# cnosdb/cnosdb

Measured on NVIDIA H100. Metric: decoded+aggregated points/s, higher is better.
Workload: dtype i64/f64

## Files before the change

cnosdb_b200/csrc/scan_kernels.cuh:

```cuda
#pragma once
#include <type_traits>

#include "cursors.cuh"

namespace tskv {

constexpr uint32_t FULL = 0xffffffffu;
constexpr int MAX_RANGES = 8;
constexpr int N_TK = 3;
constexpr int N_VK = 3;
constexpr int N_SERIAL_BINS = N_TK * N_VK;
enum { BIN_COOP_RLE_S8B = N_SERIAL_BINS, BIN_COOP_S8B_S8B = N_SERIAL_BINS + 1, BIN_COOP_RLE_GOR = N_SERIAL_BINS + 2,
       BIN_COOP_S8B_GOR = N_SERIAL_BINS + 3 };
constexpr int N_BINS = N_SERIAL_BINS + 4;

enum { TK_RLE = 0, TK_S8B = 1, TK_GEN = 2 };
enum { VK_S8B = 0, VK_GOR = 1, VK_GEN = 2 };

__host__ __device__ inline int time_class(uint8_t dk) {
  return dk == DK_RLE_SC ? TK_RLE : dk == DK_S8B_SC ? TK_S8B : TK_GEN;
}
__host__ __device__ inline int value_class(uint8_t dk) {
  return dk == DK_S8B_ZZ ? VK_S8B : dk == DK_GORILLA ? VK_GOR : VK_GEN;
}
// ... 1123 lines not shown

template <int VK>
__device__ __forceinline__ void flush_runs(const ScanParams &P, uint64_t *stab, uint64_t *stage, uint32_t &seq, bool active,
                                           uint32_t qcol, uint64_t cell, uint8_t pt, uint8_t mask, const ValueAcc<VK> &va) {
  const uint32_t m = __ballot_sync(FULL, active);
  if (m == 0) return;
  const uint32_t lane = threadIdx.x & 31;
  const uint64_t gcell = ((uint64_t)qcol << 32) | (uint32_t)cell;
  const int leader = __ffs(m) - 1;
  const uint64_t lcell = shfl_u64(gcell, leader);
  const bool same = !P.group_by_series && __all_sync(FULL, !active || gcell == lcell);
  if (same) {
    stage_partial<VK>(P, stab, stage, seq, active && va.count, va, (int)lane == leader, lcell);
  } else if (active && va.count) {
    table_update(P, stab, P.cols[qcol], cell, mask, VK == VK_GOR || (VK == VK_GEN && pt == TSKV_PT_F64), va.count, va.sum,
                 va.sum_hi, va.kmin, va.kmax);
  }
}

template <int K, typename S>
__device__ __forceinline__ bool cursor_exhausted(const DeltaCursor<K, S> &c) { return c.exhausted; }
template <bool ZZ>
__device__ __forceinline__ bool cursor_exhausted(const S8bCursor<ZZ> &c) { return c.exhausted(); }
template <int K, typename S>
__device__ __forceinline__ void cursor_reset(DeltaCursor<K, S> &c, uint32_t lane_ring) { c.bs.reset(lane_ring); }
template <bool ZZ>
__device__ __forceinline__ void cursor_reset(S8bCursor<ZZ> &c, uint32_t lane_ring) { c.reset(lane_ring); }

__device__ __forceinline__ uint32_t rle_rows_within(uint64_t d, uint64_t delta, double inv, uint32_t left) {
  const double e = (double)d * inv;
  if (e >= (double)left) return left;
  uint64_t q = (uint64_t)e;
  if (__umul64hi(q, delta) != 0 || q * delta > d) q--;
  else if (d - q * delta >= delta) q++;
  return (uint32_t)min((uint64_t)left, q + 1);
}

template <int TK, int VK, bool SEL>
__device__ __forceinline__ void scan_chunk_seg(const ScanParams &P, uint32_t item_begin, uint32_t item_end,
                                               uint32_t ring_base, uint64_t *stab, uint64_t *stage,
                                               uint32_t part, uint32_t n_parts, uint32_t part_rows) {
  const uint32_t lane = threadIdx.x & 31;
  const uint32_t item = item_begin + lane;
  const bool have_item = item < item_end;
  const uint32_t tslot = ring_base + lane * RING_LANE_STRIDE;
  const uint32_t vslot = ring_base + (TK == TK_S8B ? RING_BYTES_PER_WARP : 0) + lane * RING_LANE_STRIDE;

  uint32_t page = 0, slot = 0, qcol = 0, n_rows = 0;
  uint8_t pt = VK == VK_GOR ? TSKV_PT_F64 : TSKV_PT_I64, mask = 0;
  PageView tpv, vpv;
  S8bCursor<false> tcur;
  uint64_t rle_t0 = 0, rle_delta = 0;
  double rle_inv = 0.0;
  typename std::conditional<VK == VK_S8B, S8bCursor<true>, DeltaCursor<-1, SeqStream>>::type vcur_d;
  GorillaRing vcur_g;
  const uint32_t *vbm = nullptr;
  const uint32_t *keepw = nullptr;
  bool allnull = false;
  int64_t pend_t = 0;
  __shared__ uint4 s_tomb[SCAN_THREADS];

  if (TK == TK_S8B) tcur.reset(tslot);
  if (VK == VK_GOR) vcur_g.reset(vslot);
  else cursor_reset(vcur_d, vslot);
  uint32_t r0 = 0, page_rows = 0;
  if (have_item) {
    page = P.work_page[item];
    slot = P.work_slot[item];
    qcol = P.work_qcol[item] & 0x7f;
    const tskv_page_desc vd = P.descs[page];
    if (P.has_tomb) s_tomb[threadIdx.x] = tomb_lookup(P, vd.series_id, vd.column_id);
    const uint32_t tpage = P.time_page_of[page];
    const tskv_page_desc td = P.descs[tpage];
    if (VK != VK_GOR) pt = P.cols[qcol].phys_type;
    mask = P.cols[qcol].agg_mask;
    page_rows = vd.num_values;
    uint32_t sk_v = SKIP_NONE, sk_t = SKIP_NONE;
    bool split = false;
    if (n_parts > 1 && page_rows > part_rows) {
      sk_v = __ldg(P.skip_off + page);
      sk_t = TK == TK_S8B ? __ldg(P.skip_off + tpage) : 0u;
      split = sk_v != SKIP_NONE && sk_t != SKIP_NONE;
    }
    r0 = part * part_rows;
    tskv_status st = kind_status(vd.reserved);
    if (part != 0 && (!split || r0 >= page_rows)) {
    } else if (st != TSKV_OK) {
      report_error(P, st, page);
    } else {
      tpv.open(P.arena, td);
      vpv.open(P.arena, vd);
      n_rows = split ? min(page_rows, r0 + part_rows) : page_rows;
      vbm = reinterpret_cast<const uint32_t *>(vpv.bitset);
      if (P.row_keep) keepw = P.row_keep + P.keep_off[tpage];
      const uint32_t ent = r0 / SKIP_ROWS - 1;
      if (TK == TK_RLE) {
        DeltaCursor<DK_RLE_SC, BeStream> rc;
        st = rc.open(tpv, td.reserved);
        rle_delta = rc.delta;
        rle_t0 = rc.v + rc.delta;
        if ((int64_t)rle_delta > 0) rle_inv = 1.0 / (double)rle_delta;
      } else if (part == 0) {
        st = tcur.open(tpv, td.reserved, tslot);
      } else {
        tcur.restore(tpv, tslot, load_skip(P.skip + sk_t + ent));
      }
      if (st == TSKV_OK) {
        if (part == 0) {
          if (VK == VK_GOR) vcur_g.open(vpv, vslot);
          else { st = vcur_d.open(vpv, vd.reserved, vslot); allnull = vd.reserved == DK_ALLNULL; }
        } else {
          const SkipEntry e = load_skip(P.skip + sk_v + ent);
          if constexpr (VK == VK_GOR) vcur_g.restore(vpv, vslot, e);
          else if constexpr (VK == VK_S8B) vcur_d.restore(vpv, vslot, e);
        }
      }
      if (st == TSKV_OK && n_rows) {
        if (TK == TK_RLE) pend_t = (int64_t)(rle_t0 + (uint64_t)r0 * rle_delta);
        else if (part == 0) pend_t = (int64_t)tcur.next();
        else pend_t = (int64_t)tcur.v;
      }
      if (st != TSKV_OK) { report_error(P, st, st == TSKV_ERR_BITSET_MISMATCH ? tpage : page); n_rows = 0; }
    }
  }
  const bool to_page_end = n_rows == page_rows;
  ring_drain();

  ValueAcc<VK> va;
  va.reset();
  RunAcc acc;
  acc.first_ts = acc.last_ts = 0; acc.first_val = acc.last_val = 0; acc.first_ok = acc.last_ok = false;
  BucketState bk; bk.valid = false; bk.floor_regime = false; bk.lo = 0; bk.hi = 0; bk.idx = 0;
  bool have_run = false;
  uint32_t run_idx = 0;
  uint32_t row = r0;
  if (n_rows == 0) row = 0;
  uint32_t n_points = 0, n_inrange = 0;
  uint32_t vword = 0, vahead = vbm ? __ldg(vbm + (row >> 5)) : 0;
  uint32_t kword = 0xffffffffu;
  bool first_pending = false;
  const uint64_t flip = pt == TSKV_PT_U64 ? 0x8000000000000000ull : 0ull;
  const uint64_t group_base = P.group_by_series ? (uint64_t)slot * P.n_buckets : 0;
  uint32_t staged = 0;

  auto flush_now = [&](bool flush) {
    if (flush) va.fold(pt);
    if (SEL) {
      if (__any_sync(FULL, flush)) {
        acc.count = va.count; acc.sum = va.sum; acc.sum_hi = va.sum_hi; acc.kmin = va.kmin; acc.kmax = va.kmax;
        warp_flush<SEL>(P, stab, flush, qcol, group_base + run_idx, (int64_t)run_idx, pt, mask, acc, slot);
      }
    } else {
      flush_runs<VK>(P, stab, stage, staged, flush, qcol, group_base + run_idx, pt, mask, va);
    }
  };
  auto row_value = [&](bool accumulate, bool &vv, bool &kept) -> uint64_t {
    if ((row & 31) == 0) {
      vword = vahead;
      vahead = __ldg(vbm + (row >> 5) + 1);
      if (keepw) kword = __ldg(keepw + (row >> 5));
    }
    vv = ((vword >> (row & 31)) & 1) && !allnull;
    kept = (kword >> (row & 31)) & 1;
    uint64_t v = 0;
    if (vv) {
      v = VK == VK_GOR ? vcur_g.next() : vcur_d.next();
      n_points++;
      if (accumulate && kept) { va.count++; va.add(v, pt, flip); }
    }
    return v;
  };
  auto check_values = [&]() {
    const bool bad = VK == VK_GOR ? vcur_g.failed() : cursor_exhausted(vcur_d);
    if (bad) {
      report_error(P, (VK == VK_GOR && vcur_g.overran()) ? TSKV_ERR_SHORT_BLOCK : TSKV_ERR_BITSET_MISMATCH, page);
      n_rows = 0;
      have_run = false;
    }
  };

  uint32_t ra = 0, rb1 = 0, nb = 0xffffffffu, q32 = 0, bidx = 0;
  uint64_t e_off = 0, w_rem = 0;
  bool fast = false;
  if (TK == TK_RLE) {
    bool elig = P.n_ranges <= 1 && !P.has_tomb;
    if (elig && n_rows) {
      const uint64_t span_t = (uint64_t)(page_rows - 1) * rle_delta;
      elig = (int64_t)rle_delta > 0 && __umul64hi((uint64_t)(page_rows - 1), rle_delta) == 0 && span_t < (1ull << 62) &&
             rle_t0 + (1ull << 62) < (1ull << 63) && P.width < ((int64_t)1 << 61);
      if (elig) {
        const int64_t t0 = (int64_t)rle_t0;
        ra = 0;
        rb1 = page_rows;
        if (P.n_ranges == 1) {
          const int64_t a = P.ranges[0].min_ts, b = P.ranges[0].max_ts;
          ra = a <= t0 ? 0u : rle_rows_within((uint64_t)(a - 1) - rle_t0, rle_delta, rle_inv, page_rows);
          rb1 = b < t0 ? 0u : rle_rows_within((uint64_t)b - rle_t0, rle_delta, rle_inv, page_rows);
        }
        ra = min(max(ra, row), n_rows);
        rb1 = min(max(rb1, row), n_rows);
        if (P.width > 0 && ra < rb1) {
          const int64_t tr = (int64_t)(rle_t0 + (uint64_t)ra * rle_delta);
          if ((int64_t)((uint64_t)tr - (uint64_t)P.origin_mod + (uint64_t)P.width) < 0) {
            elig = false;
          } else if (!locate_bucket(P, tr, bk)) {
            report_error(P, TSKV_ERR_BUCKET_RANGE, page);
            n_rows = 0;
          } else {
            bidx = bk.idx;
            nb = rle_rows_within((uint64_t)bk.hi - (uint64_t)tr, rle_delta, rle_inv, 0xffffffffu);
            e_off = (uint64_t)tr + (uint64_t)nb * rle_delta - ((uint64_t)bk.hi + 1);
            q32 = rle_rows_within((uint64_t)P.width, rle_delta, rle_inv, 0xffffffffu) - 1;
            w_rem = (uint64_t)P.width - (uint64_t)q32 * rle_delta;
          }
        }
      }
    }
    fast = __all_sync(FULL, elig);
  }

  if (TK == TK_RLE && VK != VK_GEN && !SEL && fast && P.width > 0 && !P.group_by_series) {
    const bool mine = row < n_rows;
    const uint32_t with_rows = __ballot_sync(FULL, mine);
    const int src = with_rows ? __ffs(with_rows) - 1 : 0;
    const uint64_t t_first = rle_t0 + (uint64_t)row * rle_delta;
    const bool agree = (shfl_u64(rle_delta, src) == rle_delta) & (shfl_u64(t_first, src) == t_first) &
                       (shfl_u64(e_off, src) == e_off) & (__shfl_sync(FULL, row, src) == row) &
                       (__shfl_sync(FULL, n_rows, src) == n_rows) & (__shfl_sync(FULL, ra, src) == ra) &
                       (__shfl_sync(FULL, rb1, src) == rb1) & (__shfl_sync(FULL, bidx, src) == bidx) &
                       (__shfl_sync(FULL, nb, src) == nb) & (__shfl_sync(FULL, qcol, src) == qcol);
    if (with_rows && __all_sync(FULL, !mine || agree)) {
      rle_delta = shfl_u64(rle_delta, src);
      e_off = shfl_u64(e_off, src);
      w_rem = shfl_u64(w_rem, src);
      q32 = __shfl_sync(FULL, q32, src);
      row = __shfl_sync(FULL, row, src);
      ra = __shfl_sync(FULL, ra, src);
      rb1 = __shfl_sync(FULL, rb1, src);
      bidx = __shfl_sync(FULL, bidx, src);
      nb = __shfl_sync(FULL, nb, src);
      const uint64_t col = (uint64_t)__shfl_sync(FULL, qcol, src) << 32;
      uint32_t end = __shfl_sync(FULL, n_rows, src);
      while (row < end) {
        if (n_rows) {
          vword = vahead;
          vahead = __ldg(vbm + (row >> 5) + 1);
          if (keepw) kword = __ldg(keepw + (row >> 5));
        }
        const uint32_t wend = min(row + 32, end);
        const uint32_t m = (n_rows && !allnull) ? vword & (0xffffffffu >> (32 - (wend - row))) : 0u;
        const uint32_t lo = min(max(ra, row), wend) - row, hi = max(min(max(rb1, row), wend) - row, lo);
        const uint32_t take = m & kword & (uint32_t)((1ull << hi) - (1ull << lo));
        const bool dense = __all_sync(FULL, take == m);
        uint32_t r = row;
        while (r < wend) {
          const bool in = r >= ra && r < rb1;
          uint32_t pend = r < ra ? min(ra, wend) : wend;
          if (in) {
            if (nb == 0) {
              do {
                bidx++;
                nb = q32 + (e_off < w_rem ? 1u : 0u);
                e_off = e_off + (uint64_t)nb * rle_delta - (uint64_t)P.width;
              } while (nb == 0);
              if (bidx >= P.n_buckets) {
                if (n_rows) { report_error(P, TSKV_ERR_BUCKET_RANGE, page); n_rows = r; }
                end = r;
                break;
              }
            }
            const uint32_t lim = min(rb1, wend);
            pend = nb < lim - r ? r + nb : lim;
            nb -= pend - r;
          }
          const uint32_t pmask = (uint32_t)((1ull << (pend - row)) - (1ull << (r - row)));
          const uint32_t mp = n_rows ? m & pmask : 0u, tp = take & mp;
          n_points += __popc(mp);
          if (in && n_rows) n_inrange += __popc(kword & pmask);
          va.count += __popc(tp);
          if (dense) {
#pragma unroll 1
            for (uint32_t n = __popc(mp); n; n--) {
              const uint64_t v = VK == VK_GOR ? vcur_g.next() : vcur_d.next();
              va.add(v, pt, flip);
            }
          } else {
#pragma unroll 1
            for (uint32_t b = mp; b; b &= b - 1) {
              const uint64_t v = VK == VK_GOR ? vcur_g.next() : vcur_d.next();
              if (tp & b & (0u - b)) va.add(v, pt, flip);
            }
          }
          r = pend;
          if (n_rows) check_values();
          if (in && (nb == 0 || r == rb1)) {
            va.fold(pt);
            stage_partial<VK>(P, stab, stage, staged, n_rows && va.count, va, lane == 0, col | bidx);
            va.reset();
          }
        }
        row = r;
      }
      row = n_rows;
    }
  }

  const bool align = P.width > 0 && !P.group_by_series;
  bool pending = false;
  uint32_t seg_n = 0, seg_b = 0;
  bool seg_in = false, seg_masked = false;
  int64_t lim_lo = 0, lim_hi = 0;
  for (;;) {
    const bool has = row < n_rows;
    if (!__any_sync(FULL, has || have_run)) break;
    if (has && !pending) {
      pending = true;
      seg_in = false;
      seg_masked = false;
      seg_n = 0;
      if (TK == TK_RLE && fast) {
        if (row < ra) seg_n = ra - row;
        else if (row >= rb1) seg_n = n_rows - row;
        else {
          seg_in = true;
          while (nb == 0) {
            bidx++;
            nb = q32 + (e_off < w_rem ? 1u : 0u);
            e_off = e_off + (uint64_t)nb * rle_delta - (uint64_t)P.width;
          }
          if (bidx >= P.n_buckets) {
            report_error(P, TSKV_ERR_BUCKET_RANGE, page);
            seg_in = false;
            n_rows = row;
            pending = false;
          } else {
            seg_n = min(nb, rb1 - row);
            seg_b = bidx;
            if (P.width > 0) nb -= seg_n;
          }
        }
      } else {
        lim_lo = lim_hi = pend_t;
        seg_in = range_span(P, pend_t, lim_lo, lim_hi);
        if (P.has_tomb) {
          const uint4 tl = s_tomb[threadIdx.x];
          const bool dropped = tomb_span(P.tomb_ranges, P.n_tomb_global, pend_t, lim_lo, lim_hi) |
                               tomb_span(P.tomb_ranges + tl.x, tl.y, pend_t, lim_lo, lim_hi);
          seg_masked = tomb_span(P.tomb_ranges + tl.z, tl.w, pend_t, lim_lo, lim_hi);
          if (dropped) seg_in = false;
        }
        if (seg_in) {
          if (!(bk.valid && pend_t >= bk.lo && pend_t <= bk.hi) && !locate_bucket(P, pend_t, bk)) {
            report_error(P, TSKV_ERR_BUCKET_RANGE, page);
            seg_in = false;
            bk.valid = false;
            lim_lo = lim_hi = pend_t;
          } else {
            lim_lo = lim_lo > bk.lo ? lim_lo : bk.lo;
            lim_hi = lim_hi < bk.hi ? lim_hi : bk.hi;
            seg_b = bk.idx;
          }
        }
        if (TK == TK_RLE) {
          const uint32_t left = n_rows - row;
          if ((int64_t)rle_delta > 0) {
            seg_n = rle_rows_within((uint64_t)lim_hi - (uint64_t)pend_t, rle_delta, rle_inv, left);
          } else {
            int64_t t = pend_t;
            do {
              seg_n++;
              t = (int64_t)((uint64_t)t + rle_delta);
            } while (seg_n < left && t >= lim_lo && t <= lim_hi);
          }
        }
      }
    }
    bool go = pending;
    if (align) {
      const uint32_t bmin = __reduce_min_sync(FULL, (pending && seg_in) ? seg_b : 0xffffffffu);
      go = pending && (!seg_in || seg_b == bmin);
    }
    const bool newrun = go && seg_in && (!have_run || seg_b != run_idx);
    const bool flush = have_run && (newrun || !has);
    flush_now(flush);
    if (flush) have_run = false;
    if (newrun) {
      have_run = true;
      run_idx = seg_b;
      va.reset();
      if (SEL) { acc.first_ok = acc.last_ok = false; first_pending = true; }
    }
    if (go) {
      pending = false;
      const bool accumulate = seg_in && !seg_masked;
      if (TK == TK_RLE) {
        const uint32_t rend = row + seg_n;
        uint32_t r = row;
        while (r < rend) {
          if ((r & 31) == 0) {
            vword = vahead;
            vahead = __ldg(vbm + (r >> 5) + 1);
            if (keepw) kword = __ldg(keepw + (r >> 5));
          }
          const uint32_t off = r & 31;
          const uint32_t span = min(32u - off, rend - r);
          const uint32_t smask = 0xffffffffu >> (32 - span);
          const uint32_t m = allnull ? 0u : ((vword >> off) & smask);
          const uint32_t kb = (kword >> off) & smask;
          n_points += __popc(m);
          if (seg_in) n_inrange += __popc(kb);
          if (!SEL) {
            const uint32_t take = accumulate ? (m & kb) : 0u;
            va.count += __popc(take);
            if (__all_sync(__activemask(), take == m)) {
#pragma unroll 1
              for (uint32_t n = __popc(m); n; n--) {
                const uint64_t v = VK == VK_GOR ? vcur_g.next() : vcur_d.next();
                va.add(v, pt, flip);
              }
            } else {
#pragma unroll 1
              for (uint32_t b = m; b; b &= b - 1) {
                const uint64_t v = VK == VK_GOR ? vcur_g.next() : vcur_d.next();
                if (take & b & (0u - b)) va.add(v, pt, flip);
              }
            }
          } else {
            for (uint32_t j = 0; j < span; j++) {
              bool vv = (m >> j) & 1;
              uint64_t v = 0;
              if (vv) v = VK == VK_GOR ? vcur_g.next() : vcur_d.next();
              vv = vv && !seg_masked;
              if (seg_in && ((kb >> j) & 1)) {
                const int64_t t = (int64_t)(rle_t0 + (uint64_t)(r + j) * rle_delta);
                if (first_pending) { acc.first_ts = t; acc.first_val = vv ? v : 0; acc.first_ok = vv; first_pending = false; }
                acc.last_ts = t;
                acc.last_val = vv ? v : 0;
                acc.last_ok = vv;
                if (vv) { va.count++; va.add(v, pt, flip); }
              }
            }
          }
          r += span;
        }
        row = rend;
        if (!(TK == TK_RLE && fast)) pend_t = (int64_t)(rle_t0 + (uint64_t)rend * rle_delta);
      } else {
        int64_t t = pend_t;
        const uint64_t span = (uint64_t)lim_hi - (uint64_t)lim_lo;
        bool more;
#pragma unroll 1
        do {
          bool vv, kept;
          const uint64_t v = row_value(accumulate, vv, kept);
          if (SEL && seg_in && kept) {
            const bool ok = vv && !seg_masked;
            if (first_pending) { acc.first_ts = t; acc.first_val = ok ? v : 0; acc.first_ok = ok; first_pending = false; }
            acc.last_ts = t;
            acc.last_val = ok ? v : 0;
            acc.last_ok = ok;
          }
          if (seg_in && kept) n_inrange++;
          row++;
          t = (int64_t)tcur.next();
          more = row < n_rows && (uint64_t)t - (uint64_t)lim_lo <= span;
        } while (more);
        pend_t = t;
        if (tcur.exhausted() && row < n_rows) { report_error(P, TSKV_ERR_BITSET_MISMATCH, P.time_page_of[page]); n_rows = row; }
      }
      check_values();
    }
  }
  if (!SEL && staged) {
    reduce_staged<VK>(P, stab, stage, staged);
    staged = 0;
  }
  if (VK == VK_GOR && have_item && n_rows != 0 && to_page_end && vcur_g.consumed_any() && !vcur_g.drain())
    report_error(P, TSKV_ERR_SHORT_BLOCK, page);
  ring_drain();
  n_points = __reduce_add_sync(FULL, n_points);
  n_inrange = __reduce_add_sync(FULL, n_inrange);
  if (lane == 0) {
    if (n_points) atomicAdd(&P.stats[0], (unsigned long long)n_points);
    if (n_inrange) atomicAdd(&P.stats[1], (unsigned long long)n_inrange);
  }
}

#ifndef SCAN_MIN_BLOCKS
#define SCAN_MIN_BLOCKS 4
#endif
__host__ __device__ constexpr int scan_min_blocks(int , bool ) { return SCAN_MIN_BLOCKS; }
__host__ __device__ constexpr uint32_t scan_ring_bytes_per_warp(int tk) {
  return tk == TK_RLE ? RING_BYTES_PER_WARP : tk == TK_S8B ? 2 * RING_BYTES_PER_WARP : 0;
}
__host__ __device__ constexpr uint32_t scan_warp_bytes(int tk) {
  return tk == TK_GEN ? 0 : scan_ring_bytes_per_warp(tk) + FLUSH_STAGE_BYTES;
}
template <int TK, int VK, bool SEL>
__global__ void __launch_bounds__(SCAN_THREADS, scan_min_blocks(TK, SEL)) k_scan_aggregate(const __grid_constant__ ScanParams P, int bin) {
  extern __shared__ __align__(16) uint64_t s_tab[];
  if (P.use_smem) {
    for (uint32_t i = threadIdx.x; i < P.smem_words; i += SCAN_THREADS) s_tab[i] = 0;
    __syncthreads();
    for (uint32_t c = 0; c < P.n_cols; c++) {
      const ColState cs = P.cols[c];
      for (uint32_t i = threadIdx.x; i < (uint32_t)P.n_cells; i += SCAN_THREADS) {
        if (cs.agg_mask & TSKV_AGG_MIN) s_tab[cs.s_min + i] = 0x7fffffffffffffffull;
        if (cs.agg_mask & TSKV_AGG_MAX) s_tab[cs.s_max + i] = 0x8000000000000000ull;
      }
    }
    __syncthreads();
  }
  const uint32_t lane = threadIdx.x & 31;
  uint64_t *warp_area = s_tab + ((P.smem_words + 1) & ~1u) + (size_t)(threadIdx.x >> 5) * (scan_warp_bytes(TK) / 8);
  const uint32_t ring_base = (uint32_t)__cvta_generic_to_shared(warp_area);
  uint64_t *stage = warp_area + scan_ring_bytes_per_warp(TK) / 8;
  const uint32_t begin0 = __ldg(P.bin_cstart + bin), end0 = __ldg(P.bin_cstart + bin + 1);
  const uint32_t n_parts = (TK == TK_GEN || VK == VK_GEN || SEL) ? 1u : P.bin_parts[bin];
  const uint32_t part_rows = P.bin_part_rows[bin];
  const uint32_t n_chunks = ((end0 - begin0 + 31) >> 5) * n_parts;
  for (;;) {
    uint32_t c = 0;
    if (lane == 0) c = atomicAdd(P.task_counter + bin, 1u);
    c = __shfl_sync(FULL, c, 0);
    if (c >= n_chunks) break;
    const uint32_t group = n_parts > 1 ? c / n_parts : c;
    const uint32_t part = c - group * n_parts;
    const uint32_t begin = begin0 + (group << 5);
    const uint32_t end = min(begin + 32, end0);
    if constexpr (TK == TK_GEN) scan_chunk_rows<TK, VK, SEL>(P, begin, end, ring_base, s_tab);
    else scan_chunk_seg<TK, VK, SEL>(P, begin, end, ring_base, s_tab, stage, part, n_parts, part_rows);
  }
  if (P.use_smem) {
    __syncthreads();
    for (uint32_t c = 0; c < P.n_cols; c++) {
      const ColState cs = P.cols[c];
      const bool f64 = cs.phys_type == TSKV_PT_F64;
      for (uint32_t i = threadIdx.x; i < (uint32_t)P.n_cells; i += SCAN_THREADS) {
        const uint64_t cnt = s_tab[cs.s_count + i];
        if (!cnt) continue;
        atomicAdd(reinterpret_cast<unsigned long long *>(P.state + cs.count_off + i), (unsigned long long)cnt);
        if (cs.agg_mask & (TSKV_AGG_SUM | TSKV_AGG_MEAN)) {
          const uint64_t sv = s_tab[cs.s_sum + i];
          if (f64) atomicAdd(reinterpret_cast<double *>(P.state + cs.sum_off + i), __longlong_as_double((long long)sv));
          else add_int_sum(P.state + cs.sum_off + i, P.state + cs.sumhi_off + i, cs.agg_mask, sv,
                           (cs.agg_mask & TSKV_AGG_MEAN) ? (int64_t)s_tab[cs.s_hi + i] : 0);
        }
        if (cs.agg_mask & TSKV_AGG_MIN) atomicMin(reinterpret_cast<long long *>(P.state + cs.min_off + i), (long long)s_tab[cs.s_min + i]);
        if (cs.agg_mask & TSKV_AGG_MAX) atomicMax(reinterpret_cast<long long *>(P.state + cs.max_off + i), (long long)s_tab[cs.s_max + i]);
      }
    }
  }
}

struct StateLayout {
  uint64_t sum_i64_off, sum_i64_len;
  uint64_t sum_f64_off, sum_f64_len;
  uint64_t min_off, min_len;
  uint64_t max_off, max_len;
  uint64_t selval_off, selval_len;
  uint64_t first_pairs_off, first_cells;
  uint64_t last_pairs_off, last_cells;
  uint64_t first_keys_off, last_keys_off;
  uint64_t snap_off;
  uint64_t total;
};

__global__ void k_init_state(uint64_t *state, StateLayout L, unsigned long long *aux, uint32_t aux_words, uint32_t *zero32,
                             uint32_t n_zero32, uint32_t *zero32b, uint32_t n_zero32b) {
  uint64_t i = (uint64_t)blockIdx.x * blockDim.x + threadIdx.x;
  uint64_t stride = (uint64_t)gridDim.x * blockDim.x;
  for (uint64_t k = i; k < aux_words; k += stride) aux[k] = 0;
  for (uint64_t k = i; k < n_zero32; k += stride) zero32[k] = 0;
  for (uint64_t k = i; k < n_zero32b; k += stride) zero32b[k] = 0;
  for (uint64_t k = i; k < L.total; k += stride) {
    uint64_t v = 0;
    if (k >= L.min_off && k < L.min_off + L.min_len) v = 0x7fffffffffffffffull;
    else if (k >= L.max_off && k < L.max_off + L.max_len) v = 0x8000000000000000ull;
    else if (k >= L.first_pairs_off && k < L.first_pairs_off + 2 * L.first_cells) v = ((k - L.first_pairs_off) & 1) ? 0 : 0x7fffffffffffffffull;
    else if (k >= L.last_pairs_off && k < L.last_pairs_off + 2 * L.last_cells) v = ((k - L.last_pairs_off) & 1) ? 0 : 0x8000000000000000ull;
    state[k] = v;
  }
}

struct MeanExport {
  uint64_t lo_off, hi_off, dst_off;
  uint32_t is_signed, pad;
};

__global__ void k_export_pairs(uint64_t *state, StateLayout L, const MeanExport *means, uint32_t n_means,
                               uint64_t n_cells) {
  uint64_t i = (uint64_t)blockIdx.x * blockDim.x + threadIdx.x;
  uint64_t stride = (uint64_t)gridDim.x * blockDim.x;
  for (uint32_t m = 0; m < n_means; m++) {
    const MeanExport me = means[m];
    for (uint64_t k = i; k < n_cells; k += stride) {
      uint64_t lo = state[me.lo_off + k];
      int64_t hi = (int64_t)state[me.hi_off + k];
      double d;
      if (me.is_signed) d = (double)(((__int128)hi << 64) + (__int128)(unsigned __int128)lo);
      else d = (double)(((unsigned __int128)(uint64_t)hi << 64) | (unsigned __int128)lo);
      state[me.dst_off + k] = (uint64_t)__double_as_longlong(d);
    }
  }
  for (uint64_t k = i; k < L.first_cells; k += stride) {
    state[L.first_keys_off + k] = state[L.first_pairs_off + 2 * k];
// ... 151 lines not shown
```

cnosdb_b200/csrc/tskv_gpu.cu:

```cuda
#include <algorithm>
#include <cmath>
#include <atomic>
#include <cstdio>
#include <cstdlib>
#include <cstring>
#include <mutex>
#include <string>
#include <thread>
#include <vector>

#include <cuda_runtime.h>
#include <dlfcn.h>
#include <nccl.h>

#include "host_util.h"
#include "decode_kernels.cuh"
#include "skip_kernels.cuh"
#include "merge_kernels.cuh"

using namespace tskv;

#define CU_TRY(ctx, expr)                                                              \
  do {                                                                                 \
    cudaError_t e__ = (expr);                                                          \
// ... 1152 lines not shown
      }
      if (q->n_time_ranges > 0) {
        int64_t qlo = q->time_ranges[0].min_ts, qhi = q->time_ranges[0].max_ts;
        for (uint32_t k = 1; k < q->n_time_ranges; k++) {
          qlo = std::min(qlo, q->time_ranges[k].min_ts);
          qhi = std::max(qhi, q->time_ranges[k].max_ts);
        }
        lo = std::max(lo, qlo);
        hi = std::min(hi, qhi);
      }
      if (hi < lo) {
        rel_bits = 0;
      } else {
        uint64_t span = (uint64_t)hi - (uint64_t)lo;
        rel_bits = bits_for(span);
        rel_base = lo;
      }
    }
    if (rel_bits + slot_bits > 62) {
      ctx->set_error("first/last across series: (bucket width or time span) x series count does not fit the 62-bit tie-break key");
      delete s;
      return TSKV_ERR_UNSUPPORTED;
    }
  }

  std::vector<ColState> cols(q->n_columns);
  StateLayout &sl = s->sl;
  uint64_t off = 0;
  sl.sum_i64_off = off;
  for (uint32_t c = 0; c < q->n_columns; c++) {
    const tskv_agg_column &qc = q->columns[c];
    cols[c] = ColState{};
    cols[c].column_id = qc.column_id;
    cols[c].phys_type = qc.phys_type;
    cols[c].agg_mask = qc.agg_mask;
    cols[c].count_off = off;
    off += n_cells;
    if ((qc.agg_mask & (TSKV_AGG_SUM | TSKV_AGG_MEAN)) && qc.phys_type != TSKV_PT_F64) {
      cols[c].sum_off = off;
      off += n_cells;
    }
  }
  sl.sum_i64_len = off - sl.sum_i64_off;
  sl.sum_f64_off = off;
  for (uint32_t c = 0; c < q->n_columns; c++)
    if ((q->columns[c].agg_mask & (TSKV_AGG_SUM | TSKV_AGG_MEAN)) && q->columns[c].phys_type == TSKV_PT_F64) {
      cols[c].sum_off = off;
      off += n_cells;
    }
  std::vector<MeanExport> means;
  std::vector<uint64_t> msum_off(q->n_columns, 0);
  for (uint32_t c = 0; c < q->n_columns; c++)
    if ((q->columns[c].agg_mask & TSKV_AGG_MEAN) && q->columns[c].phys_type != TSKV_PT_F64) {
      msum_off[c] = off;
      off += n_cells;
    }
  sl.sum_f64_len = off - sl.sum_f64_off;
  uint64_t n_first = 0, n_last = 0;
  for (uint32_t c = 0; c < q->n_columns; c++) {
    if (q->columns[c].agg_mask & TSKV_AGG_FIRST) n_first += n_cells;
    if (q->columns[c].agg_mask & TSKV_AGG_LAST) n_last += n_cells;
  }
  sl.first_cells = n_first;
  sl.last_cells = n_last;
  sl.min_off = off;
  for (uint32_t c = 0; c < q->n_columns; c++)
    if (q->columns[c].agg_mask & TSKV_AGG_MIN) {
      cols[c].min_off = off;
      off += n_cells;
    }
  sl.first_keys_off = off;
  off += n_first;
  sl.min_len = off - sl.min_off;
  sl.max_off = off;
  for (uint32_t c = 0; c < q->n_columns; c++)
    if (q->columns[c].agg_mask & TSKV_AGG_MAX) {
      cols[c].max_off = off;
      off += n_cells;
    }
  sl.last_keys_off = off;
  off += n_last;
  sl.max_len = off - sl.max_off;
  sl.selval_off = off;
  off += n_first + n_last;
  sl.selval_len = n_first + n_last;
  off = (off + 1) & ~1ull;
  sl.first_pairs_off = off;
  {
    uint64_t o = off;
    for (uint32_t c = 0; c < q->n_columns; c++)
      if (q->columns[c].agg_mask & TSKV_AGG_FIRST) {
        cols[c].first_off = o;
        o += 2 * n_cells;
      }
    off = o;
  }
  sl.last_pairs_off = off;
  {
    uint64_t o = off;
    for (uint32_t c = 0; c < q->n_columns; c++)
      if (q->columns[c].agg_mask & TSKV_AGG_LAST) {
        cols[c].last_off = o;
        o += 2 * n_cells;
      }
    off = o;
  }
  sl.snap_off = off;
  off += n_first + n_last;
  for (uint32_t c = 0; c < q->n_columns; c++)
    if (msum_off[c]) {
      cols[c].sumhi_off = off;
      means.push_back(MeanExport{cols[c].sum_off, off, msum_off[c], q->columns[c].phys_type == TSKV_PT_I64 ? 1u : 0u, 0});
      off += n_cells;
    }
  sl.total = off;

  std::vector<OutCol> outs;
  {
    uint64_t fk = sl.first_keys_off, lk = sl.last_keys_off, fv = sl.selval_off, lv = sl.selval_off + n_first;
    for (uint32_t c = 0; c < q->n_columns; c++) {
      const tskv_agg_column &qc = q->columns[c];
      for (unsigned bit = 0; bit < 7; bit++) {
        unsigned agg = 1u << bit;
        if (!(qc.agg_mask & agg)) continue;
        OutCol oc{};
        oc.count_off = cols[c].count_off;
        oc.agg = (uint8_t)agg;
        oc.phys_type = qc.phys_type;
        switch (agg) {
          case TSKV_AGG_SUM: oc.src_off = cols[c].sum_off; break;
          case TSKV_AGG_MEAN: oc.src_off = msum_off[c] ? msum_off[c] : cols[c].sum_off; break;
          case TSKV_AGG_MIN: oc.src_off = cols[c].min_off; break;
          case TSKV_AGG_MAX: oc.src_off = cols[c].max_off; break;
          case TSKV_AGG_FIRST: oc.src_off = fk; oc.val_off = fv; break;
          case TSKV_AGG_LAST: oc.src_off = lk; oc.val_off = lv; break;
          default: break;
        }
        outs.push_back(oc);
      }
      if (qc.agg_mask & TSKV_AGG_FIRST) { fk += n_cells; fv += n_cells; }
      if (qc.agg_mask & TSKV_AGG_LAST) { lk += n_cells; lv += n_cells; }
    }
  }

  const uint32_t n_items = pages->n_items;
  s->ctx = ctx;
  cudaEventCreate(&s->ev0);
  cudaEventCreate(&s->ev1);
  for (int b = 0; b <= N_BINS; b++) cudaEventCreate(&s->ev_bin[b]);
  for (int b = 0; b < N_BINS; b++) {
    cudaEventCreate(&s->ev_bin_start[b]);
    cudaEventCreate(&s->ev_bin_done[b]);
    cudaEventCreateWithFlags(&s->ev_gather[b], cudaEventDisableTiming);
  }
  s->n_series_sel = q->series_ids ? q->n_series : 0;
  s->n_blocks = (n_items + 1023) / 1024;
  cudaError_t e = cudaSuccess;
  uint64_t h2d = 0;
  if (q->series_ids) {
    e = stream_alloc(ctx, &s->d_series, q->n_series);
    if (e == cudaSuccess && q->n_series)
      e = cudaMemcpyAsync(s->d_series, q->series_ids, (size_t)q->n_series * 4, cudaMemcpyHostToDevice, ctx->stream);
    h2d += (uint64_t)q->n_series * 4;
  }
  if (e == cudaSuccess && q->series_ids) e = stream_alloc(ctx, &s->d_rank_slot, pages->series.size());
  if (e == cudaSuccess) e = stream_alloc(ctx, &s->d_bucket, (size_t)2 * N_BINS * q->n_columns + 1);
  {
    const char *wl = getenv("TSKV_WORKLIST");
    s->worklist_by_items = wl ? wl[0] == 'i' : (uint64_t)pages->n_cg > 32ull * std::max<uint64_t>(1, pages->series.size());
  }
  if (e == cudaSuccess) e = stream_alloc(ctx, &s->d_cg_slot, pages->n_cg);
  if (e == cudaSuccess) e = stream_alloc(ctx, &s->d_item_flag, n_items);
  if (e == cudaSuccess) e = stream_alloc(ctx, &s->d_block_count, s->n_blocks);
  if (e == cudaSuccess) e = stream_alloc(ctx, &s->d_work_page, n_items);
  if (e == cudaSuccess) e = stream_alloc(ctx, &s->d_work_slot, n_items);
  if (e == cudaSuccess) e = stream_alloc(ctx, &s->d_work_qcol, n_items);
  if (e == cudaSuccess) e = stream_alloc(ctx, &s->d_bin_cstart, N_BINS + 2);
  if (e == cudaSuccess) e = stream_alloc(ctx, &s->d_cols, cols.size());
  if (e == cudaSuccess) e = stream_alloc(ctx, &s->d_outs, outs.size());
  s->n_means = (uint32_t)means.size();
  if (e == cudaSuccess) e = stream_alloc(ctx, &s->d_means, means.size());
  if (e == cudaSuccess && !means.empty())
    e = cudaMemcpyAsync(s->d_means, means.data(), means.size() * sizeof(MeanExport), cudaMemcpyHostToDevice, ctx->stream);
  if (e == cudaSuccess) e = stream_alloc(ctx, &s->d_state, sl.total);
  s->preds.n = q->n_predicates;
  for (uint32_t k = 0; k < q->n_predicates; k++) s->preds.p[k] = q->predicates[k];
  if (q->n_predicates) ensure_page_stats(ctx, pages);
  if (e == cudaSuccess && q->n_predicates) e = stream_alloc(ctx, &s->d_row_keep, (size_t)pages->keep_words);
  if (e == cudaSuccess) e = stream_alloc(ctx, reinterpret_cast<unsigned long long **>(&s->d_task_counter), 32);
  if (e == cudaSuccess) e = stream_alloc(ctx, &s->d_values, L.n_out * L.n_cells);
  if (e == cudaSuccess) e = stream_alloc(ctx, &s->d_validity, L.validity_bytes + 8);
  if (e == cudaSuccess) e = cudaMemcpyAsync(s->d_outs, outs.data(), outs.size() * sizeof(OutCol), cudaMemcpyHostToDevice, ctx->stream);
  h2d += cols.size() * sizeof(ColState) + outs.size() * sizeof(OutCol) + means.size() * sizeof(MeanExport) + sizeof(ScanParams);
  if (e != cudaSuccess) {
    ctx->set_error(std::string("scan_prepare: ") + cudaGetErrorString(e));
    free_scan(s);
    return e == cudaErrorMemoryAllocation ? TSKV_ERR_OOM : TSKV_ERR_CUDA;
  }
  unsigned long long *aux = reinterpret_cast<unsigned long long *>(s->d_task_counter);
  s->d_status = reinterpret_cast<int32_t *>(aux + 8);
  s->d_err_page = aux + 9;
  s->d_stats = aux + 10;
  s->d_counters = aux + 12;
  s->d_crc_status = reinterpret_cast<int32_t *>(aux + 28);
  s->d_crc_err_page = aux + 29;
  cudaEventCreateWithFlags(&s->ev_crc, cudaEventDisableTiming);
  cudaEventCreateWithFlags(&s->ev_ccrc, cudaEventDisableTiming);

  ScanParams &P = s->params;
  P.arena = pages->d_arena;
  P.descs = pages->d_descs;
  P.time_page_of = pages->d_time_page_of;
  P.work_page = s->d_work_page;
  P.work_slot = s->d_work_slot;
  P.work_qcol = s->d_work_qcol;
  P.bin_cstart = s->d_bin_cstart;
  P.cols = s->d_cols;
  P.state = s->d_state;
  P.task_counter = s->d_task_counter;
  P.status = s->d_status;
  P.err_page = s->d_err_page;
  P.stats = s->d_stats;
  P.n_ranges = q->n_time_ranges;
  for (uint32_t k = 0; k < q->n_time_ranges; k++) P.ranges[k] = q->time_ranges[k];
  if (q->n_time_ranges) {
    ensure_time_bounds(ctx, pages);
    s->prune.n = q->n_time_ranges;
    for (uint32_t k = 0; k < q->n_time_ranges; k++) s->prune.r[k] = q->time_ranges[k];
  }
  P.width = q->width;
  P.origin_mod = q->width > 0 ? q->origin % q->width : 0;
  P.first_bucket_start = q->first_bucket_start;
  P.n_buckets = q->n_buckets;
  P.group_by_series = q->group_by_series;
  P.n_cells = n_cells;
  P.slot_bits = slot_bits;
  P.slot_max = slot_bits ? (uint32_t)((1ull << slot_bits) - 1) : 0;
  P.rel_base = rel_base;
  {
    uint32_t words = 0;
    for (uint32_t c = 0; c < q->n_columns; c++) {
      const uint8_t m = q->columns[c].agg_mask;
      const bool is_int = q->columns[c].phys_type != TSKV_PT_F64;
      cols[c].s_count = words; words += (uint32_t)n_cells;
      if (m & (TSKV_AGG_SUM | TSKV_AGG_MEAN)) { cols[c].s_sum = words; words += (uint32_t)n_cells; }
      if ((m & TSKV_AGG_MEAN) && is_int) { cols[c].s_hi = words; words += (uint32_t)n_cells; }
      if (m & TSKV_AGG_MIN) { cols[c].s_min = words; words += (uint32_t)n_cells; }
      if (m & TSKV_AGG_MAX) { cols[c].s_max = words; words += (uint32_t)n_cells; }
      if (n_cells > (1u << 20)) { words = UINT32_MAX / 2; break; }
    }
    const char *lim_env = getenv("TSKV_SMEM_TABLE_KB");
    const uint64_t limit = (lim_env ? (uint64_t)atoi(lim_env) : 32) * 1024;
    P.use_smem = (!q->group_by_series && (uint64_t)words * 8 <= limit) ? 1u : 0u;
    P.smem_words = P.use_smem ? words : 0;
    P.n_cols = q->n_columns;
    P.row_keep = s->d_row_keep;
    P.keep_off = pages->d_keep_off;
    P.skip_off = pages->d_skip_off;
    P.skip = pages->d_skip;
    for (int b = 0; b < N_BINS; b++) { P.bin_parts[b] = 1; P.bin_part_rows[b] = 0; }
    P.has_tomb = pages->n_tomb_ranges ? 1u : 0u;
    P.tomb_keys = pages->d_tomb_keys;
    P.tomb_off = pages->d_tomb_off;
    P.tomb_ranges = pages->d_tomb_ranges;
    P.n_tomb_keys = pages->n_tomb_keys;
    P.n_tomb_global = pages->n_tomb_global;
    s->tomb_epoch = pages->tomb_epoch;
  }
  if (cudaMemcpyAsync(s->d_cols, cols.data(), cols.size() * sizeof(ColState), cudaMemcpyHostToDevice, ctx->stream) != cudaSuccess) {
    ctx->set_error("scan_prepare: column table upload failed");
    free_scan(s);
    return TSKV_ERR_CUDA;
  }

  {
    const char *mode = getenv("TSKV_COOP");
    const double sel_frac = plan_selected_fraction(pages->series.data(), pages->series.size(), q->series_ids, q->n_series);
    const double est_total = (double)pages->n_items * sel_frac;
    for (int b = N_SERIAL_BINS; b < N_BINS; b++)
      s->use_coop[b] = (pages->n_tomb_ranges || q->n_predicates) ? false
                       : mode             ? (mode[0] == '1')
                                          : false;
    (void)est_total;
    uint32_t gor_group = 1;
    {
      double est_gor = 0;
      for (int b = N_SERIAL_BINS; b < N_BINS; b++)
        if (is_gor_coop_bin(b) && s->use_coop[b]) est_gor += (pages->h_bin_start[b + 1] - pages->h_bin_start[b]) * sel_frac;
      int gocc = 0;
      const void *gfn = coop_kernel_for(BIN_COOP_RLE_GOR, s->has_sel);
      cudaOccupancyMaxActiveBlocksPerMultiprocessor(&gocc, gfn, SCAN_THREADS, coop_smem_bytes(BIN_COOP_RLE_GOR, P.smem_words));
      const double resident_warps = (double)ctx->sm_count * std::max(1, gocc) * (SCAN_THREADS / 32);
      gor_group = plan_gorilla_group(est_gor, resident_warps);
      if (const char *g = getenv("TSKV_GOR_GROUP")) gor_group = (uint32_t)std::min(32, std::max(1, atoi(g)));
      s->coop.gor_group = gor_group;
    }
    uint32_t parts[N_BINS];
    for (int b = 0; b < N_BINS; b++) parts[b] = 1;
    if (pages->d_skip && !s->has_sel) {
      double est_chunks = 0;
      for (int b = 0; b < N_BINS; b++) est_chunks += std::ceil((pages->h_bin_start[b + 1] - pages->h_bin_start[b]) * sel_frac / 32.0);
      const double resident_warps = (double)ctx->sm_count * SCAN_MIN_BLOCKS * (SCAN_THREADS / 32);
      const char *pt_env = getenv("TSKV_PARTS_TARGET");
      uint32_t want = plan_parts_wanted(est_chunks, resident_warps, pt_env ? atof(pt_env) : 4.0);
      const char *parts_env = getenv("TSKV_PARTS");
      if (parts_env) want = (uint32_t)std::max(1, atoi(parts_env));
      for (int b = 0; b < N_BINS; b++) {
        const int sb = serial_bin_of(b);
        if (s->use_coop[b] || sb / N_VK == TK_GEN || sb % N_VK == VK_GEN) continue;
        uint32_t want_b = want;
        if (sb / N_VK == TK_S8B) {
          const char *ts_env = getenv("TSKV_PARTS_TS");
          if (ts_env) want_b = (uint32_t)std::max(1, atoi(ts_env));
        }
        uint32_t part_rows = 0;
        parts[b] = plan_bin_parts(pages->h_bin_maxrows[b], SKIP_ROWS, want_b, &part_rows);
        P.bin_parts[b] = parts[b];
        P.bin_part_rows[b] = part_rows;
      }
    }
    double w[N_BINS], wsum = 0, need_sum = 0, occ_weighted = 0;
    int need[N_BINS] = {0}, occ_bin[N_BINS] = {0};
    for (int b = 0; b < N_BINS; b++) {
      uint32_t n_bin = pages->h_bin_start[b + 1] - pages->h_bin_start[b];
      w[b] = n_bin * bin_cost(b, s->use_coop[b]);
      wsum += w[b];
      if (!n_bin) continue;
      int occ = 0;
      if (!s->use_coop[b]) {
        const int sb = serial_bin_of(b);
        const void *fn = (const void *)(s->has_sel ? scan_kernel_for<true>(sb) : scan_kernel_for<false>(sb));
        cudaOccupancyMaxActiveBlocksPerMultiprocessor(&occ, s->has_sel ? scan_kernel_for<true>(sb) : scan_kernel_for<false>(sb),
                                                      SCAN_THREADS, serial_smem_bytes(sb, P.smem_words));
      } else {
        const void *fn = coop_kernel_for(b, s->has_sel);
        cudaOccupancyMaxActiveBlocksPerMultiprocessor(&occ, fn, SCAN_THREADS, coop_smem_bytes(b, P.smem_words));
      }
      occ = std::max(1, occ);
      occ_bin[b] = occ;
      const double est_items = n_bin * sel_frac * 1.02 + 32;
      const uint32_t per_task = !s->use_coop[b] ? 32u : is_gor_coop_bin(b) ? gor_group : 1u;
      const double tasks = est_items / per_task * parts[b];
      need[b] = (int)(tasks / (SCAN_THREADS / 32)) + 1;
      need[b] = std::min(need[b], (int)(((uint64_t)(n_bin + per_task - 1) / per_task * parts[b] + SCAN_THREADS / 32 - 1) / (SCAN_THREADS / 32)));
      need_sum += need[b];
      occ_weighted += (double)need[b] * occ;
    }
    const double capacity = need_sum > 0 ? (occ_weighted / need_sum) * ctx->sm_count : 0;
    bool any_coop = false;
    for (int b = N_SERIAL_BINS; b < N_BINS; b++) any_coop |= s->use_coop[b] && need[b];
    if (need_sum <= capacity) {
      for (int b = 0; b < N_BINS; b++)
        if (need[b]) s->grid[b] = std::max(1, need[b]);
    } else if (!any_coop) {
      double chunks[N_BINS], t_chunk[N_BINS];
      for (int b = 0; b < N_BINS; b++) {
        const uint32_t n_bin = pages->h_bin_start[b + 1] - pages->h_bin_start[b];
        chunks[b] = need[b] ? std::ceil((n_bin * sel_frac * 1.02 + 16) / 32.0) * parts[b] : 0;
        t_chunk[b] = n_bin ? chunk_cost(b) * ((double)pages->h_bin_rows[b] / n_bin / parts[b] + 12.0) : 1.0;
      }
      plan_serial_grids(N_BINS, chunks, t_chunk, occ_bin, ctx->sm_count, SCAN_THREADS / 32, s->grid);
      for (int b = 0; b < N_BINS; b++) s->grid[b] = std::min(s->grid[b], std::max(need[b], 0));
      {
        const char *ov = getenv("TSKV_GRID_OVERSUB");
        const double f = ov ? atof(ov) : 4.0;
        if (f > 1.0)
          for (int b = 0; b < N_BINS; b++) s->grid[b] = std::min(std::max(need[b], 0), (int)std::ceil(s->grid[b] * f));
      }
      const char *gm = getenv("TSKV_GRID_MODE");
      if (gm && gm[0] == '1')
        for (int b = 0; b < N_BINS; b++) s->grid[b] = need[b];
    } else {
      bool fixed[N_BINS] = {false};
      double cap_left = capacity, w_left = 0;
      for (int b = 0; b < N_BINS; b++) w_left += need[b] ? w[b] : 0;
      for (int round = 0; round < N_BINS; round++) {
        bool changed = false;
        for (int b = 0; b < N_BINS; b++) {
          if (!need[b] || fixed[b]) continue;
          if (need[b] <= cap_left * w[b] / w_left) {
            s->grid[b] = std::max(1, need[b]);
            fixed[b] = true;
            cap_left -= s->grid[b];
            w_left -= w[b];
            changed = true;
          }
        }
        if (!changed) break;
      }
      for (int b = 0; b < N_BINS; b++)
        if (need[b] && !fixed[b]) s->grid[b] = std::max(1, std::min(need[b], (int)(cap_left * w[b] / w_left + 0.5)));
    }
    for (int b = N_SERIAL_BINS; b < N_BINS; b++) {
      if (!is_gor_coop_bin(b) || !s->use_coop[b] || !s->grid[b]) continue;
      const int k = b == BIN_COOP_RLE_GOR ? 0 : 1;
      const size_t words = (size_t)s->grid[b] * (SCAN_THREADS / 32) * gor_group * GOR_REC_STRIDE;
      if (stream_alloc(ctx, &s->d_gor_scratch[k], words) != cudaSuccess) {
        ctx->set_error("scan_prepare: out of memory for the gorilla record scratch");
        free_scan(s);
        return TSKV_ERR_OOM;
      }
      s->coop.gor_scratch[k] = s->d_gor_scratch[k];
    }
    if (q->width > 0) {
      s->coop.div = make_magic((uint64_t)q->width);
      const int64_t d0 = (int64_t)((uint64_t)q->first_bucket_start - (uint64_t)P.origin_mod + (uint64_t)q->width);
      s->coop.grid_ok = (d0 >= 0 && d0 % q->width == 0) ? 1u : 0u;
      s->coop.q0 = s->coop.grid_ok ? d0 / q->width : 0;
    }
  }
  s->chunk_epoch = pages->chunk_epoch;
  if (pages->merge_rows) {
    const OverlapPlan &op = pages->overlap;
    const size_t n_mcg = op.mcg_cg.size();
    std::vector<uint8_t> active(n_mcg, 0);
    std::vector<uint32_t> mpage;
    std::vector<uint64_t> mrow_off, mbm_off;
    for (size_t k = 0; k < n_mcg; k++) {
      const uint32_t cg = op.mcg_cg[k], tp = pages->h_cg_time_page[cg];
      const tskv_page_desc &td = pages->h_descs[tp];
      if (q->series_ids && !std::binary_search(q->series_ids, q->series_ids + q->n_series, td.series_id)) continue;
      if (q->n_time_ranges) {
        bool overlaps = false;
        for (uint32_t r = 0; r < q->n_time_ranges; r++)
          overlaps = overlaps || (pages->h_cg_bounds[cg].min_ts <= q->time_ranges[r].max_ts && pages->h_cg_bounds[cg].max_ts >= q->time_ranges[r].min_ts);
        if (!overlaps) continue;
      }
      bool any = false;
      for (uint64_t p = (uint64_t)tp + 1; p < pages->n_descs && pages->h_descs[p].phys_type != TSKV_PT_TIME; p++)
        for (uint32_t c = 0; c < q->n_columns; c++)
          if (pages->h_descs[p].column_id == q->columns[c].column_id) {
            if (pages->h_descs[p].phys_type != q->columns[c].phys_type) {
              ctx->set_error("page type does not match the query column type", (int64_t)p);
              free_scan(s);
              return TSKV_ERR_INVALID_ARG;
            }
            any = true;
            mpage.push_back((uint32_t)p);
            mrow_off.push_back((uint64_t)c * pages->merge_rows + op.mcg_row0[k]);
            mbm_off.push_back(((uint64_t)c * pages->merge_bm_words + pages->h_mcg_bm0[k]) * 4);
            s->merge_page_bytes += pages->h_descs[p].size;
          }
      if (!any) continue;
      active[k] = 1;
      s->merge_page_bytes += td.size;
      s->merge_read_pages++;
    }
    s->n_merge_pages = (uint32_t)mpage.size();
    s->merge_read_pages += mpage.size();
    cudaError_t me = stream_alloc(ctx, &s->d_mcg_active, n_mcg);
    if (me == cudaSuccess) me = cudaMemcpyAsync(s->d_mcg_active, active.data(), n_mcg, cudaMemcpyHostToDevice, ctx->stream);
    if (me == cudaSuccess) me = stream_alloc(ctx, &s->d_mvals, (size_t)q->n_columns * pages->merge_rows);
    if (me == cudaSuccess) me = stream_alloc(ctx, &s->d_mvalid, (size_t)q->n_columns * pages->merge_bm_words);
    if (me == cudaSuccess) me = stream_alloc(ctx, &s->d_mpage, mpage.size());
    if (me == cudaSuccess) me = stream_alloc(ctx, &s->d_mrow_off, mpage.size());
    if (me == cudaSuccess) me = stream_alloc(ctx, &s->d_mbm_off, mpage.size());
    if (me == cudaSuccess && !mpage.empty()) {
      me = cudaMemcpyAsync(s->d_mpage, mpage.data(), mpage.size() * 4, cudaMemcpyHostToDevice, ctx->stream);
      if (me == cudaSuccess) me = cudaMemcpyAsync(s->d_mrow_off, mrow_off.data(), mpage.size() * 8, cudaMemcpyHostToDevice, ctx->stream);
      if (me == cudaSuccess) me = cudaMemcpyAsync(s->d_mbm_off, mbm_off.data(), mpage.size() * 8, cudaMemcpyHostToDevice, ctx->stream);
    }
    if (me == cudaSuccess) me = cudaStreamSynchronize(ctx->stream);
    if (me != cudaSuccess) {
      ctx->set_error(std::string("scan_prepare (merge pass): ") + cudaGetErrorString(me));
      free_scan(s);
      return me == cudaErrorMemoryAllocation ? TSKV_ERR_OOM : TSKV_ERR_CUDA;
    }
    h2d += n_mcg + mpage.size() * 20;
    MergeParams &M = s->merge;
    M.ts = pages->d_merge_ts;
    M.mcg_row0 = pages->d_mcg_row0;
    M.mcg_cg = pages->d_mcg_cg;
    M.mcg_stream = pages->d_mcg_stream;
    M.stream_group = pages->d_stream_group;
    M.stream_first_mcg = pages->d_stream_first_mcg;
    M.group_first_stream = pages->d_group_first_stream;
    M.mcg_active = s->d_mcg_active;
    M.vals = s->d_mvals;
    M.valid = s->d_mvalid;
    M.mcg_bm0 = pages->d_mcg_bm0;
    M.cg_time_page = pages->d_cg_time_page;
    M.cg_slot = s->d_cg_slot;
    M.n_rows = pages->merge_rows;
    M.bm_words = pages->merge_bm_words;
    M.n_mcg = (uint32_t)n_mcg;
    M.sel = s->has_sel ? 1u : 0u;
  }
  ctx->counters.h2d_bytes = h2d;
  *out_scan = s;
  return TSKV_OK;
}

static tskv_status enqueue_scan(tskv_ctx *ctx, tskv_scan *s, bool capturing = false) {
  const tskv_pages *pages = s->pages;
  const uint32_t n_items = pages->n_items;
  if (s->tomb_epoch != pages->tomb_epoch) {
    ctx->set_error("the page set's tombstones changed after this scan was prepared", -1);
    return TSKV_ERR_INVALID_ARG;
  }
  if (s->chunk_epoch != pages->chunk_epoch) {
    ctx->set_error("the page set's chunk files changed after this scan was prepared", -1);
    return TSKV_ERR_INVALID_ARG;
  }
  if (!capturing) cudaEventRecord(s->ev0, ctx->stream);
  unsigned long long *aux = reinterpret_cast<unsigned long long *>(s->d_task_counter);
  uint64_t launches = 0;
  {
    const uint32_t init_blocks = (uint32_t)std::min<uint64_t>((s->sl.total + 255) / 256, 4096);
    k_init_state<<<std::max(1u, init_blocks), 256, 0, ctx->stream>>>(s->d_state, s->sl, aux, 32, s->d_bin_cstart, N_BINS + 2, s->d_bucket,
                                                                   N_BINS * s->n_cols);
    launches++;
  }
  const bool need_cg_slot = s->worklist_by_items || s->preds.n || (s->merge.n_rows && s->n_merge_pages);
  if (pages->n_cg && need_cg_slot) {
    if (s->d_rank_slot) {
      CU_TRY(ctx, cudaMemsetAsync(s->d_rank_slot, 0xff, pages->series.size() * 4, ctx->stream));
      if (s->n_series_sel) {
        k_select_ids<<<(s->n_series_sel + 255) / 256, 256, 0, ctx->stream>>>(pages->d_series_sorted, (uint32_t)pages->series.size(), s->d_series,
                                                                         s->n_series_sel, s->d_rank_slot);
        launches++;
      }
    }
    k_select_cg<<<(pages->n_cg + 255) / 256, 256, 0, ctx->stream>>>(pages->n_cg, s->d_rank_slot, pages->d_cg_series_rank, s->d_cg_slot);
    launches++;
  }
  if (s->preds.n && pages->n_cg) {
    k_row_filter<<<(pages->n_cg + 127) / 128, 128, 0, ctx->stream>>>(pages->h_mapped ? pages->h_mapped : pages->d_arena, pages->d_descs,
                                                                     pages->n_descs, pages->d_cg_time_page, pages->n_cg, s->d_cg_slot,
                                                                     s->preds, pages->d_keep_off, s->d_row_keep, s->d_status, s->d_err_page);
    launches++;
  }
  if (n_items && s->worklist_by_items) {
    k_flag_items<<<s->n_blocks, 1024, 0, ctx->stream>>>(pages->d_descs, pages->d_item_info,
                                                        pages->d_cg_time_page, n_items, s->d_cg_slot, s->d_cols,
                                                        s->n_cols, pages->d_bin_start, s->d_item_flag,
                                                        s->d_block_count, s->d_counters, s->d_status,
                                                        s->prune.n ? pages->d_cg_bounds : nullptr, s->prune, pages->d_cg_merge,
                                                        s->preds.n ? pages->d_page_stats : nullptr, s->preds, pages->n_descs, pages->n_cg);
    k_scan_blocks<<<1, 1024, 0, ctx->stream>>>(s->d_block_count, s->n_blocks, s->d_bin_cstart + N_BINS + 1);
    k_scatter_items<<<s->n_blocks, 1024, 0, ctx->stream>>>(pages->d_item_page, pages->d_item_cg, n_items, s->d_item_flag,
                                                           s->d_block_count, s->d_cg_slot, pages->d_bin_start,
                                                           s->d_work_page, s->d_work_slot, s->d_work_qcol,
                                                           s->d_bin_cstart, s->d_bin_cstart + N_BINS + 1);
    launches += 3;
  } else if (n_items) {
    WorkListArgs A{};
    A.descs = pages->d_descs;
    A.n_descs = pages->n_descs;
    A.cg_time_page = pages->d_cg_time_page;
    A.n_cg = pages->n_cg;
    A.rank_cg_start = pages->d_rank_cg_start;
    A.rank_cg = pages->d_rank_cg;
    A.page_bin = pages->d_page_bin;
    A.set_series = pages->d_series_sorted;
    A.n_set_series = (uint32_t)pages->series.size();
    A.series_ids = s->d_series;
    A.n_sel = s->d_series ? s->n_series_sel : (uint32_t)pages->series.size();
    A.cols = s->d_cols;
    A.n_cols = s->n_cols;
    A.cg_bounds = s->prune.n ? pages->d_cg_bounds : nullptr;
    A.prune = s->prune;
    A.cg_merge = pages->d_cg_merge;
    A.page_stats = s->preds.n ? pages->d_page_stats : nullptr;
    A.preds = s->preds;
    const uint32_t n_buckets = N_BINS * s->n_cols;
    A.bucket_count = s->d_bucket;
    A.bucket_off = s->d_bucket + n_buckets;
    A.work_page = s->d_work_page;
    A.work_slot = s->d_work_slot;
    A.work_qcol = s->d_work_qcol;
    A.counters = s->d_counters;
    A.status = s->d_status;
    const uint32_t wblocks = std::max(1u, (A.n_sel + WL_THREADS - 1) / WL_THREADS);
    if (A.n_sel) k_worklist_count<<<wblocks, WL_THREADS, n_buckets * 4, ctx->stream>>>(A);
    k_worklist_offsets<<<1, 256, 0, ctx->stream>>>(s->d_bucket, s->d_bucket + n_buckets, s->n_cols, s->d_bin_cstart);
    if (A.n_sel) k_worklist_emit<<<wblocks, WL_THREADS, 2 * n_buckets * 4, ctx->stream>>>(A);
    launches += 3;
  }
  if (s->merge.n_rows && s->n_merge_pages) {
    CU_TRY(ctx, cudaMemsetAsync(s->d_mvalid, 0, (size_t)s->n_cols * s->merge.bm_words * 4, ctx->stream));
    const uint32_t dblocks = (uint32_t)(((uint64_t)s->n_merge_pages * 32 + DECODE_THREADS - 1) / DECODE_THREADS);
    k_decode_warp<<<dblocks, DECODE_THREADS, 0, ctx->stream>>>(pages->h_mapped ? pages->h_mapped : pages->d_arena, pages->d_descs, 0, s->d_mpage,
                                                              s->n_merge_pages, s->d_mrow_off, s->d_mbm_off, s->d_mvals,
                                                              reinterpret_cast<uint8_t *>(s->d_mvalid), s->d_status, s->d_err_page, s->d_stats);
    const uint32_t mblocks = (uint32_t)((s->merge.n_rows + 127) / 128);
    k_merge_chunks<<<mblocks, 128, 0, ctx->stream>>>(s->params, s->merge);
    launches += 2;
  }
  cudaEvent_t ev_fork = capturing ? s->ev_cfork : s->ev_bin[0];
  cudaEventRecord(ev_fork, ctx->stream);
  int order[N_BINS];
  for (int b = 0; b < N_BINS; b++) order[b] = b;
  static const bool gather_concurrent = getenv("TSKV_GATHER_CONCURRENT") != nullptr;
  if (pages->h_mapped && !gather_concurrent)
    std::stable_sort(order, order + N_BINS, [&](int a, int b) { return pages->h_bin_bytes[a] > pages->h_bin_bytes[b]; });
  else if (!pages->h_mapped)
    std::stable_sort(order, order + N_BINS, [&](int a, int b) { return chunk_cost(a) > chunk_cost(b); });
  int prev_gather = -1;
  bool crc_forked = false;
  for (int oi = 0; oi < N_BINS; oi++) {
    const int b = order[oi];
    if (!s->grid[b]) continue;
    cudaStreamWaitEvent(ctx->bin_stream[b], ev_fork, 0);
    int bin = b;
    if (pages->h_mapped) {
      if (prev_gather >= 0 && !gather_concurrent) cudaStreamWaitEvent(ctx->bin_stream[b], s->ev_gather[prev_gather], 0);
      uint32_t n_bin = pages->h_bin_start[b + 1] - pages->h_bin_start[b];
// ... 296 lines not shown
```

Measured before the change: 115.9 billion.

## Add warp-uniform bucket-walk fast path for S8B time columns with fixed-width windows

Adds a specialized path for simple-8b time pages with non-generic value encodings, no selection, no tombstones and at most one time range. Each warp skips rows before the range, agrees on a common starting bucket, and then walks fixed-width buckets in order. When the validity bitmap is all set, it accumulates values in a tight loop without per-row null or keep checks. Partials are staged once per bucket. The default parts target also drops from 4 to 2, so fewer partitions are made per bin, trading parallelism for less per-partition overhead.

```diff
diff --git a/cnosdb_b200/csrc/scan_kernels.cuh b/cnosdb_b200/csrc/scan_kernels.cuh
--- a/cnosdb_b200/csrc/scan_kernels.cuh
+++ b/cnosdb_b200/csrc/scan_kernels.cuh
@@ -1449,6 +1449,87 @@
         row = r;
       }
       row = n_rows;
+    }
+  }
+
+  if (TK == TK_S8B && VK != VK_GEN && !SEL && P.width > 0 && P.width < ((int64_t)1 << 61) && !P.group_by_series &&
+      !P.has_tomb && P.n_ranges <= 1) {
+    const int64_t ta = P.n_ranges ? P.ranges[0].min_ts : INT64_MIN, tb = P.n_ranges ? P.ranges[0].max_ts : INT64_MAX;
+    if (row < n_rows && pend_t < ta) {
+#pragma unroll 1
+      do {
+        bool vv, kept;
+        row_value(false, vv, kept);
+        row++;
+        pend_t = (int64_t)tcur.next();
+      } while (row < n_rows && pend_t < ta);
+      if (tcur.exhausted() && row < n_rows) { report_error(P, TSKV_ERR_BITSET_MISMATCH, P.time_page_of[page]); n_rows = row; }
+      check_values();
+    }
+    const bool inr = row < n_rows && pend_t <= tb;
+    const bool ok = inr && locate_bucket(P, pend_t, bk) && bk.floor_regime;
+    const uint32_t bmin = __reduce_min_sync(FULL, ok ? bk.idx : 0xffffffffu);
+    const uint32_t lead = __ballot_sync(FULL, ok && bk.idx == bmin);
+    const int src = lead ? __ffs(lead) - 1 : 0;
+    int64_t lo = (int64_t)shfl_u64((uint64_t)bk.lo, src), hi = (int64_t)shfl_u64((uint64_t)bk.hi, src);
+    const uint32_t c = __shfl_sync(FULL, qcol, src);
+    if (lead && __all_sync(FULL, !inr || (ok && bk.idx - bmin <= 1 && qcol == c))) {
+      const uint64_t col = (uint64_t)c << 32;
+      const int64_t hi_cap = INT64_MAX - 2 * P.width;
+      bool dense = !keepw;
+      if (row < n_rows) {
+        dense = dense && !allnull;
+        const uint32_t w1 = (n_rows - 1) >> 5;
+#pragma unroll 1
+        for (uint32_t wi = row >> 5; dense && wi <= w1; wi++) {
+          uint32_t x = __ldg(vbm + wi);
+          if (wi == row >> 5) x |= (1u << (row & 31)) - 1u;
+          if (wi == w1 && (n_rows & 31)) x |= 0xffffffffu << (n_rows & 31);
+          dense = x == 0xffffffffu;
+        }
+      }
+      dense = __all_sync(FULL, dense);
+      for (uint32_t b = bmin;; b++) {
+        const bool more = row < n_rows && pend_t <= tb;
+        const uint32_t where = __reduce_or_sync(FULL, more ? (pend_t < lo ? 4u : pend_t <= hi ? 2u : 1u) : 0u);
+        if (where != 2u && where != 3u) break;
+        if (b >= P.n_buckets || hi > hi_cap) break;
+        const uint64_t span = (uint64_t)(hi < tb ? hi : tb) - (uint64_t)lo;
+        if (more && (uint64_t)pend_t - (uint64_t)lo <= span) {
+          int64_t t = pend_t;
+          if (dense) {
+            const uint32_t r1 = row;
+#pragma unroll 1
+            do {
+              const uint64_t v = VK == VK_GOR ? vcur_g.next() : vcur_d.next();
+              va.add(v, pt, flip);
+              row++;
+              t = (int64_t)tcur.next();
+            } while (row < n_rows && (uint64_t)t - (uint64_t)lo <= span);
+            va.count += row - r1;
+            n_points += row - r1;
+            n_inrange += row - r1;
+          } else {
+#pragma unroll 1
+            do {
+              bool vv, kept;
+              row_value(true, vv, kept);
+              if (kept) n_inrange++;
+              row++;
+              t = (int64_t)tcur.next();
+            } while (row < n_rows && (uint64_t)t - (uint64_t)lo <= span);
+          }
+          pend_t = t;
+          if (tcur.exhausted() && row < n_rows) { report_error(P, TSKV_ERR_BITSET_MISMATCH, P.time_page_of[page]); n_rows = row; }
+          check_values();
+        }
+        va.fold(pt);
+        stage_partial<VK>(P, stab, stage, staged, n_rows && va.count, va, lane == 0, col | b);
+        va.reset();
+        lo = hi + 1;
+        hi += P.width;
+      }
+      if (dense) vword = vahead = 0xffffffffu;
     }
   }
 
diff --git a/cnosdb_b200/csrc/tskv_gpu.cu b/cnosdb_b200/csrc/tskv_gpu.cu
--- a/cnosdb_b200/csrc/tskv_gpu.cu
+++ b/cnosdb_b200/csrc/tskv_gpu.cu
@@ -1478,7 +1478,7 @@
       for (int b = 0; b < N_BINS; b++) est_chunks += std::ceil((pages->h_bin_start[b + 1] - pages->h_bin_start[b]) * sel_frac / 32.0);
       const double resident_warps = (double)ctx->sm_count * SCAN_MIN_BLOCKS * (SCAN_THREADS / 32);
       const char *pt_env = getenv("TSKV_PARTS_TARGET");
-      uint32_t want = plan_parts_wanted(est_chunks, resident_warps, pt_env ? atof(pt_env) : 4.0);
+      uint32_t want = plan_parts_wanted(est_chunks, resident_warps, pt_env ? atof(pt_env) : 2.0);
       const char *parts_env = getenv("TSKV_PARTS");
       if (parts_env) want = (uint32_t)std::max(1, atoi(parts_env));
       for (int b = 0; b < N_BINS; b++) {
```

Result: faster. 123.2 billion (median of 6 runs) (+6.3%).
